# nuclia/nucliadb

Measured on AMD Instinct MI355X. Metric: queries/sec + recall@10 (768-dim cosine k-NN, HNSW M=30 ef=30 ef_upper=4 build_ef_upper=4, k=10), higher is better.
Workload: dtype f32

## Files before the change

### include/nidx_gpu.h

```cpp
#ifndef NIDX_GPU_H
#define NIDX_GPU_H

#include <stddef.h>
#include <stdint.h>

#ifdef __cplusplus
extern "C" {
#endif

#define NIDX_OK 0
#define NIDX_ERR_IO (-1)
#define NIDX_ERR_INCONSISTENT_DIMENSIONS (-2)
#define NIDX_ERR_INVALID_CONFIGURATION (-3)
#define NIDX_ERR_EMPTY_MERGE (-4)
#define NIDX_ERR_INVALID_ARGUMENT (-5)
#define NIDX_ERR_UNSUPPORTED (-6)
#define NIDX_ERR_DEVICE (-7)
#define NIDX_ERR_INVALID_GRAPH (-8)
#define NIDX_ERR_INEXACT (-9)
#define NIDX_ERR_OUT_OF_MEMORY (-10)
#define NIDX_ERR_INTERNAL (-11)
#define NIDX_ERR_BUSY (-12)

int32_t nidx_gpu_last_error(char *buf, size_t len);
// ... 168 lines not shown
int32_t nidx_gpu_vector_search_filtered_per_query(nidx_gpu_vector_index_t *index, const float *queries, uint32_t n_queries,
                                                  uint32_t query_dimension, const nidx_gpu_vector_search_params_t *params,
                                                  const nidx_gpu_filter_program_t *programs, uint32_t n_filters,
                                                  const uint32_t *filter_of_query, uint32_t *out_segment, uint32_t *out_paragraph,
                                                  uint32_t *out_vector, float *out_score, uint32_t *out_count, int32_t *out_method,
                                                  uint64_t *out_matching);

int32_t nidx_gpu_vector_segment_search_device(nidx_gpu_vector_index_t *index, uint32_t segment,
                                              const float *d_queries, uint32_t n_queries,
                                              const nidx_gpu_vector_search_params_t *params,
                                              const uint64_t *d_filter, uint32_t *d_out_vector,
                                              float *d_out_score, uint32_t *d_out_count, uint32_t *d_stats,
                                              void *stream);

int32_t nidx_gpu_vector_device_flags(nidx_gpu_vector_index_t *index, void *stream, uint32_t *flags_out);

int32_t nidx_gpu_vector_segment_search_device_exact(nidx_gpu_vector_index_t *index, uint32_t segment, const float *d_queries,
                                                    uint32_t n_queries, const nidx_gpu_vector_search_params_t *params,
                                                    const uint64_t *d_filter, uint32_t *d_out_block, uint32_t *host_out_block,
                                                    void *stream, uint32_t *n_retried_out);

int32_t nidx_gpu_diag_gather(const float *d_rows, uint32_t n_rows, uint32_t dimension, uint32_t waves, uint32_t gathers_per_wave,
                             int32_t rows_in_flight, uint32_t repeats, float *ms_out);

int32_t nidx_gpu_diag_single_query_latency(nidx_gpu_vector_index_t *index, const float *queries, uint32_t n_queries, uint32_t dimension,
                                           const nidx_gpu_vector_search_params_t *params, uint32_t threads, uint32_t calls,
                                           float *latencies_us_out, double *elapsed_s_out);

int32_t nidx_gpu_vector_search_submit(nidx_gpu_vector_index_t *index, const float *queries, uint32_t n_queries, uint32_t query_dimension,
                                      const nidx_gpu_vector_search_params_t *params, const uint64_t *const *segment_filters,
                                      uint64_t *ticket_out);
int32_t nidx_gpu_vector_search_wait(nidx_gpu_vector_index_t *index, uint64_t ticket, uint32_t *out_segment, uint32_t *out_paragraph,
                                    uint32_t *out_vector, float *out_score, uint32_t *out_count, uint32_t *n_retried_out);
int32_t nidx_gpu_vector_search_submit_filtered_per_query(nidx_gpu_vector_index_t *index, const float *queries, uint32_t n_queries,
                                                         uint32_t query_dimension, const nidx_gpu_vector_search_params_t *params,
                                                         const nidx_gpu_filter_program_t *programs, uint32_t n_filters,
                                                         const uint32_t *filter_of_query, uint64_t *ticket_out);

int32_t nidx_gpu_vector_search_submit_filtered_per_query_async(nidx_gpu_vector_index_t *index, const float *queries, uint32_t n_queries,
                                                               uint32_t query_dimension, const nidx_gpu_vector_search_params_t *params,
                                                               const nidx_gpu_filter_program_t *programs, uint32_t n_filters,
                                                               const uint32_t *filter_of_query, uint64_t *ticket_out);
int32_t nidx_gpu_vector_search_wait_routed(nidx_gpu_vector_index_t *index, uint64_t ticket, uint32_t *out_segment, uint32_t *out_paragraph,
                                           uint32_t *out_vector, float *out_score, uint32_t *out_count, int32_t *out_method,
                                           uint64_t *out_matching, uint32_t *n_retried_out);
int32_t nidx_gpu_use_hnsw_threshold(uint64_t total_nodes, uint64_t top_k, int32_t has_rabitq, uint64_t *threshold_out);
// ... 532 lines not shown
```

### nucliadb_amd/_lib.py

```python
from __future__ import annotations

import ctypes as C
import os

_HERE = os.path.dirname(os.path.abspath(__file__))
LIB_PATH = os.environ.get("NIDX_GPU_LIB") or os.path.join(_HERE, "libnidx_gpu.so")

NIDX_OK = 0
NIDX_ERR_IO = -1
NIDX_ERR_INCONSISTENT_DIMENSIONS = -2
NIDX_ERR_INVALID_CONFIGURATION = -3
NIDX_ERR_EMPTY_MERGE = -4
NIDX_ERR_INVALID_ARGUMENT = -5
NIDX_ERR_UNSUPPORTED = -6
NIDX_ERR_DEVICE = -7
NIDX_ERR_INVALID_GRAPH = -8
NIDX_ERR_INEXACT = -9
NIDX_ERR_OUT_OF_MEMORY = -10
NIDX_ERR_INTERNAL = -11
NIDX_ERR_BUSY = -12

SIMILARITY_DOT, SIMILARITY_COSINE = 0, 1
METHOD_AUTO, METHOD_HNSW, METHOD_BRUTE_FORCE, METHOD_BRUTE_FORCE_MFMA, METHOD_BRUTE_FORCE_BF16 = 0, 1, 2, 3, 4
METHOD_RABITQ_HNSW, METHOD_RABITQ_BRUTE_FORCE = 5, 6
# ... 306 lines not shown
    "nidx_gpu_vector_generation": (C.c_int32, [C.c_void_p, C.POINTER(C.c_uint64)]),
    "nidx_gpu_vector_set_tunable": (C.c_int32, [C.c_void_p, C.c_char_p, C.c_int32]),
    "nidx_gpu_vector_space_usage": (C.c_int32, [C.c_void_p, C.POINTER(C.c_uint64)]),
    "nidx_gpu_vector_num_segments": (C.c_int32, [C.c_void_p, C.POINTER(C.c_uint32)]),
    "nidx_gpu_vector_segment_records": (C.c_int32, [C.c_void_p, C.c_uint32, C.POINTER(C.c_uint32)]),
    "nidx_gpu_vector_search": (C.c_int32, [C.c_void_p, C.c_void_p, C.c_uint32, C.POINTER(VectorSearchParamsC), C.c_void_p,
                                           C.c_void_p, C.c_void_p, C.c_void_p, C.c_void_p, C.c_void_p, C.c_void_p]),
    "nidx_gpu_vector_search_dim": (C.c_int32, [C.c_void_p, C.c_void_p, C.c_uint32, C.c_uint32, C.POINTER(VectorSearchParamsC),
                                               C.c_void_p, C.c_void_p, C.c_void_p, C.c_void_p, C.c_void_p, C.c_void_p, C.c_void_p]),
    "nidx_gpu_vector_set_filter_index": (C.c_int32, [C.c_void_p, C.c_uint32, C.POINTER(FilterIndexC)]),
    "nidx_gpu_vector_search_filtered": (C.c_int32, [C.c_void_p, C.c_void_p, C.c_uint32, C.c_uint32, C.POINTER(VectorSearchParamsC),
                                                    C.c_void_p, C.c_void_p, C.c_void_p, C.c_void_p, C.c_void_p, C.c_void_p, C.c_void_p,
                                                    C.c_void_p]),
    "nidx_gpu_vector_segment_search_device": (C.c_int32, [C.c_void_p, C.c_uint32, C.c_void_p, C.c_uint32,
                                                          C.POINTER(VectorSearchParamsC), C.c_void_p, C.c_void_p, C.c_void_p,
                                                          C.c_void_p, C.c_void_p, C.c_void_p]),
    "nidx_gpu_bm25_apply_deletions": (C.c_int32, [C.c_void_p, C.c_uint32, C.c_void_p, C.c_uint32, C.POINTER(C.c_uint64)]),
    "nidx_gpu_vector_set_filter_keys": (C.c_int32, [C.c_void_p, C.c_uint32, C.c_void_p, C.c_void_p, C.c_uint32]),
    "nidx_gpu_vector_lookup_filter_keys": (C.c_int32, [C.c_void_p, C.c_uint32, C.c_void_p, C.c_void_p, C.c_void_p, C.c_uint32, C.c_void_p, C.c_void_p]),
    "nidx_gpu_diag_single_query_latency": (C.c_int32, [C.c_void_p, C.c_void_p, C.c_uint32, C.c_uint32, C.POINTER(VectorSearchParamsC), C.c_uint32,
                                                       C.c_uint32, C.c_void_p, C.POINTER(C.c_double)]),
    "nidx_gpu_diag_gather": (C.c_int32, [C.c_void_p, C.c_uint32, C.c_uint32, C.c_uint32, C.c_uint32, C.c_int32, C.c_uint32,
                                         C.POINTER(C.c_float)]),
    "nidx_gpu_vector_device_flags": (C.c_int32, [C.c_void_p, C.c_void_p, C.POINTER(C.c_uint32)]),
    "nidx_gpu_vector_segment_search_device_exact": (C.c_int32, [C.c_void_p, C.c_uint32, C.c_void_p, C.c_uint32,
                                                                C.POINTER(VectorSearchParamsC), C.c_void_p, C.c_void_p, C.c_void_p,
                                                                C.c_void_p, C.POINTER(C.c_uint32)]),
    "nidx_gpu_vector_search_one": (C.c_int32, [C.c_void_p, C.c_void_p, C.c_uint32, C.POINTER(VectorSearchParamsC), C.c_void_p,
                                               C.c_void_p, C.c_void_p, C.c_void_p, C.POINTER(C.c_uint32)]),
    "nidx_gpu_vector_search_submit": (C.c_int32, [C.c_void_p, C.c_void_p, C.c_uint32, C.c_uint32, C.POINTER(VectorSearchParamsC), C.c_void_p,
                                                  C.POINTER(C.c_uint64)]),
    "nidx_gpu_vector_search_wait": (C.c_int32, [C.c_void_p, C.c_uint64, C.c_void_p, C.c_void_p, C.c_void_p, C.c_void_p, C.c_void_p,
                                                C.POINTER(C.c_uint32)]),
    "nidx_gpu_vector_search_filtered_per_query": (C.c_int32, [C.c_void_p, C.c_void_p, C.c_uint32, C.c_uint32, C.POINTER(VectorSearchParamsC),
                                                              C.c_void_p, C.c_uint32, C.c_void_p, C.c_void_p, C.c_void_p, C.c_void_p,
                                                              C.c_void_p, C.c_void_p, C.c_void_p, C.c_void_p]),
    "nidx_gpu_vector_search_submit_filtered_per_query": (C.c_int32, [C.c_void_p, C.c_void_p, C.c_uint32, C.c_uint32,
                                                                     C.POINTER(VectorSearchParamsC), C.c_void_p, C.c_uint32, C.c_void_p,
                                                                     C.POINTER(C.c_uint64)]),
    "nidx_gpu_vector_search_submit_filtered_per_query_async": (C.c_int32, [C.c_void_p, C.c_void_p, C.c_uint32, C.c_uint32,
                                                                           C.POINTER(VectorSearchParamsC), C.c_void_p, C.c_uint32, C.c_void_p,
                                                                           C.POINTER(C.c_uint64)]),
    "nidx_gpu_vector_search_wait_routed": (C.c_int32, [C.c_void_p, C.c_uint64, C.c_void_p, C.c_void_p, C.c_void_p, C.c_void_p, C.c_void_p,
                                                       C.c_void_p, C.c_void_p, C.POINTER(C.c_uint32)]),
    "nidx_gpu_use_hnsw_threshold": (C.c_int32, [C.c_uint64, C.c_uint64, C.c_int32, C.POINTER(C.c_uint64)]),
    "nidx_gpu_vector_routed_stats": (C.c_int32, [C.c_void_p, C.POINTER(VectorRoutedStatsC)]),
# ... 195 lines not shown
```

### nucliadb_amd/csrc/hnsw_device.h

```cpp
#pragma once
#include "device_common.h"
#include "kernels.h"

namespace nidx {

#define NIDX_POOL_CAP 512
#define NIDX_VIS_EMPTY 0xffffffffu
#define NIDX_DEFER_CAP 256

struct NbBuf {
    uint32_t addr[64];
    float ab[64];
    float xx[64];
};
struct SearchShared {
    uint64_t pool[NIDX_POOL_CAP];
    NbBuf nb[2];
    uint32_t eps[256];
    int ctrl[12];
};

template <int NJ>
struct QueryRegs {
    float4 qv[NJ];
    float qq;
    double sqrt_qq;
};

template <int NJ>
__device__ inline void load_query(QueryRegs<NJ> &q, const float *qrow, uint32_t dp, int lane, bool cosine) {
    float acc = 0.f;
#pragma unroll
    for (int j = 0; j < NJ; j++) {
        q.qv[j] = load_row_chunk(qrow, dp, j, lane);
        acc = fma4(q.qv[j], q.qv[j], acc);
    }
    q.qq = wave_butterfly_sum(acc);
    q.sqrt_qq = cosine ? sqrt((double)q.qq) : 0.0;
}

__device__ inline float score_from_sums(float ab, float xx, float qq, double sqrt_qq, bool cosine) {
    if (!cosine) return ab;
    double dab = (double)ab, dxx = (double)xx;
// ... 224 lines not shown
template <int NJ, int EVR>
__device__ inline void eval_neighbours(const SegDev &seg, const QueryRegs<NJ> &q, NbBuf &nb, int n, bool cosine) {
    const int lane = threadIdx.x & 63;
    const int wave = nidx_tid() >> 6;
    const int nwaves = blockDim.x >> 6;
    for (int base = wave * EVR; base < n; base += nwaves * EVR) eval_row_group<NJ, EVR>(seg, q, nb, base, n, cosine, lane);
}

template <int NJ, int EVR>
__device__ inline void eval_neighbours_dynamic(const SegDev &seg, const QueryRegs<NJ> &q, NbBuf &nb, int n, bool cosine, int *next_row) {
    const int lane = threadIdx.x & 63;
    for (;;) {
        int base = 0;
        if (lane == 0) base = atomicAdd(next_row, EVR);
        base = __builtin_amdgcn_readfirstlane(base);
        if (base >= n) break;
        eval_row_group<NJ, EVR>(seg, q, nb, base, n, cosine, lane);
    }
}

#define NIDX_CMD_EVAL 0
#define NIDX_CMD_CLEAR 1
#define NIDX_CMD_EXIT 2
__device__ inline void split_post(SearchShared &sh, int op, int p, int n, int lane) {
    if (lane == 0) {
        sh.ctrl[0] = op | (p << 2) | (n << 3);
        sh.ctrl[3] = 0;
    }
    lds_barrier();
}
__device__ inline void split_close() { lds_barrier(); }
__device__ inline uint32_t load_edge_word(const GraphDev &g, uint32_t node, int layer, int lane, uint32_t &deg) {
    uint32_t w = 0;
    if (layer == 0) {
        w = g.l0[(size_t)node * NIDX_L0_STRIDE + lane];
    } else {
        uint32_t base = g.upper_base[node];
        if (base != 0xffffffffu && lane < NIDX_UP_STRIDE) w = g.upper[((size_t)base + (layer - 1)) * NIDX_UP_STRIDE + lane];
    }
    deg = lane_bcast_u32(w, 0);
    return w;
}

template <int NJ, int EVR>
__device__ inline void split_worker_loop(const SegDev &seg, const QueryRegs<NJ> &q, SearchShared &sh, uint32_t *vis, uint32_t vis_cap, bool cosine) {
    for (;;) {
        lds_barrier();
        const int cmd = __builtin_amdgcn_readfirstlane(sh.ctrl[0]);
        const int op = cmd & 3;
        if (op == NIDX_CMD_EVAL) eval_neighbours_dynamic<NJ, EVR>(seg, q, sh.nb[(cmd >> 2) & 1], cmd >> 3, cosine, &sh.ctrl[3]);
        else if (op == NIDX_CMD_CLEAR) vis_clear(vis, vis_cap);
        lds_barrier();
        if (op == NIDX_CMD_EXIT) return;
    }
}

#define NIDX_PARK_SLOTS 4
#define NIDX_EPS_BARE 0
#define NIDX_EPS_PARKED 1
#define NIDX_EPS_CARRIED 2
template <int NJ, int EFL, int EVR, bool SPLIT = false>
__device__ inline void layer_search_block(const SegDev &seg, const GraphDev &g, int layer, int k,
                                          const QueryRegs<NJ> &q, SearchShared &sh, uint32_t *vis, uint32_t vis_log2,
                                          WaveTopK<EFL> &res, SearchCounters &st, int ep_mode = NIDX_EPS_BARE) {
    const int lane = threadIdx.x & 63;
    const bool ctl = SPLIT ? true : (nidx_tid() >> 6) == 0;
    const bool cosine = seg.similarity == 1;
    const uint32_t vis_cap = 1u << vis_log2;
    const bool carried = ep_mode == NIDX_EPS_CARRIED;
    int pool_len = 0;
    uint32_t vis_count = 0;

    if constexpr (SPLIT) {
        split_post(sh, NIDX_CMD_CLEAR, 0, 0, lane);
        vis_clear(vis, vis_cap);
        split_close();
    } else {
        vis_clear(vis, vis_cap);
        __syncthreads();
    }
    int n_new = sh.ctrl[2];
    if (n_new > k) k = n_new < 64 * EFL ? n_new : 64 * EFL;
    CandSet<EFL> cand;
    cand.init();
    const int n_eps = carried ? 0 : n_new;
    uint32_t ptag = 0xffffffffu, pbase = 0xffffffffu;
// ... 196 lines not shown
            }
            if constexpr (SPLIT) split_post(sh, NIDX_CMD_EVAL, p ^ 1, n_next_reg, lane);
            else lds_barrier();
            const uint64_t t_b = clock64();
            st.cyc_ctl += t_b - t_a;
            const bool has_next = SPLIT ? false : sh.ctrl[5] != 0;
            const int n_next = SPLIT ? n_next_reg : sh.ctrl[6 + (p ^ 1)];
            if (!ctl && has_next) eval_neighbours_dynamic<NJ, EVR>(seg, q, nb_next, n_next, cosine, &sh.ctrl[3]);
            if (ctl) {
                while (todo) {
                    float ws = res.worst_score();
                    if (res.len >= k) {
                        todo &= __ballot(s > ws);
                        if (!todo) break;
                    }
                    int j = __ffsll((long long)todo) - 1;
                    todo &= ~(1ull << j);
                    float sj = lane_bcast_f32(s, j);
                    if (sj > ws || res.len < k) {
                        uint64_t ek;
                        bool eu;
                        cand.insert(res, rank_key(sj, lane_bcast_u32(addr, j)), k, lane, ek, eu);
                        if (eu && ek != NIDX_EMPTY_KEY && !(rank_key_score(ek) < res.worst_score())) {
                            if (pool_len == NIDX_POOL_CAP) {
                                pool_prune(sh.pool, pool_len, res.worst_score(), lane);
                                if (pool_len == NIDX_POOL_CAP) {
                                    st.flags |= NIDX_FLAG_POOL_INEXACT;
                                    pool_len--;
                                }
                            }
                            if (lane == 0) sh.pool[pool_len] = ek;
                            pool_len++;
                        }
                    }
                }
                int redo = 0;
                cont = 0;
                if (overflow) {
                    st.flags |= NIDX_FLAG_VISITED_OVERFLOW;
                } else {
                    cur = cand.pop(res);
                    if (cur == NIDX_EMPTY_KEY && pool_len > 0) cur = pool_pop(sh.pool, pool_len, lane);
                    cont = cur != NIDX_EMPTY_KEY && !(rank_key_score(cur) < res.worst_score());
                    redo = cont && cur != nxt;
                }
                redo_reg = redo;
                if (!SPLIT && lane == 0) {
                    sh.ctrl[0] = cont;
                    sh.ctrl[4] = redo;
// ... 42 lines not shown
```

### nucliadb_amd/csrc/hnsw_search.hip

```cpp
#include "hnsw_device.h"

namespace nidx {

template <int NJ>
__device__ inline bool rows_equal(const SegDev &seg, uint32_t a, uint32_t b, int lane) {
    const float *ra = seg.vectors + (size_t)a * seg.dp, *rb = seg.vectors + (size_t)b * seg.dp;
    bool eq = true;
#pragma unroll
    for (int j = 0; j < NJ; j++) {
        uint32_t e = (uint32_t)j * 256u + (uint32_t)lane * 4u;
        if (e < seg.dp) {
            uint4 x = *reinterpret_cast<const uint4 *>(ra + e);
            uint4 y = *reinterpret_cast<const uint4 *>(rb + e);
            eq = eq && x.x == y.x && x.y == y.y && x.z == y.z && x.w == y.w;
        }
    }
    return __all(eq);
}

template <int NJ, int EVR, int EFL, bool SPLIT>
__device__ __forceinline__ void hnsw_search_body(const HnswSearchArgs &a, const uint32_t qi, unsigned char *smem) {
    SearchShared &sh = *reinterpret_cast<SearchShared *>(smem);
    uint32_t *vis = reinterpret_cast<uint32_t *>(smem + sizeof(SearchShared));
    __shared__ uint32_t res_addr[64 * EFL];
    __shared__ float res_score[64 * EFL];
    __shared__ uint32_t res_para[64 * EFL];

    const int lane = threadIdx.x & 63;
    const bool cosine = a.seg.similarity == 1;
    const int k = (int)a.k;

    QueryRegs<NJ> q;
    load_query<NJ>(q, a.queries + (size_t)qi * a.seg.dp, a.seg.dp, lane, cosine);
    if constexpr (SPLIT) {
        if ((nidx_tid() >> 6) != 0) {
            split_worker_loop<NJ, EVR>(a.seg, q, sh, vis, 1u << a.vis_log2, cosine);
            return;
        }
    }
    const bool ctl = SPLIT ? true : (nidx_tid() >> 6) == 0;
    const uint64_t *filter = a.filter;
    if (a.filter_row) {
        const uint32_t row = a.filter_row[qi];
        filter = row == NIDX_FILTER_ROW_NONE ? nullptr : a.filter_table + (size_t)row * a.filter_words;
    }

    SearchCounters st = {0, 0, 0, 0, 0, 0, 0};
    const uint64_t t_start = clock64();
    WaveTopK<EFL> res;
// ... 25 lines not shown
                    a.dump_score[(size_t)qi * NIDX_DUMP_STRIDE + e] = rank_key_score(key);
                }
            }
            if (lane == 0) {
                a.dump_count[qi] = (uint32_t)res.len;
                if (a.stats) a.stats[(size_t)qi * NIDX_STAT_STRIDE + NIDX_STAT_FLAGS] = st.flags;
                if (st.flags && a.flag_word) atomicOr(a.flag_word, st.flags);
                if (a.flag_rows) a.flag_rows[qi] = st.flags;
            }
        }
        if constexpr (SPLIT) {
            split_post(sh, NIDX_CMD_EXIT, 0, 0, lane);
            split_close();
        }
        return;
    }

    const uint32_t vis_cap = 1u << a.vis_log2;
    int n_res = 0;
    bool scan_done = false;
    if (a.stats == nullptr && !entry_mode) {
        if (ctl) {
            bool done = false;
            if (res.len > 0 && st.flags == 0 && sh.ctrl[2] <= ef && ef + NIDX_DEFER_CAP <= NIDX_POOL_CAP) {
                const float s0 = rank_key_score(res.at(0)), ws = res.worst_score();
                if (s0 == s0 && ws == ws) {
                    uint32_t mp[EFL], mok[EFL];
#pragma unroll
                    for (int i = 0; i < EFL; i++) {
                        mp[i] = 0;
                        mok[i] = 0;
                        if (64 * i + lane < res.len) {
                            const uint32_t c = rank_key_addr(res.mine(i));
                            const uint32_t p = a.seg.para_of_vec ? a.seg.para_of_vec[c] : c;
                            mp[i] = p;
                            mok[i] = (!a.seg.alive || bit_test(a.seg.alive, p)) && (!filter || bit_test(filter, p));
                        }
                    }
                    int expansions = 0;
                    for (int r = 0; r < res.len; r++) {
                        const uint64_t ck = res.at(r);
                        const float cs = rank_key_score(ck);
                        const uint32_t c = rank_key_addr(ck);
                        if (!(cs > ws)) break;
                        if (cs < a.min_score) {
                            done = true;
                            break;
// ... 61 lines not shown
            const uint32_t addr = a.entry_vec[(size_t)qi * k + i];
            vis_insert(vis, a.vis_log2, addr);
            sh.pool[i] = rank_key(a.entry_score[(size_t)qi * k + i], addr);
        }
        pool_len = n_entry;
        vis_count = n_entry;
        if (lane == 0) {
            sh.ctrl[9] = -1;
            sh.ctrl[10] = 0;
        }
    } else if (ctl && !from_set) {
#pragma unroll
        for (int i = 0; i < EFL; i++) {
            uint64_t key = res.mine(i);
            if (64 * i + lane < res.len) {
                vis_insert(vis, a.vis_log2, rank_key_addr(key));
                sh.pool[64 * i + lane] = key;
            }
        }
        pool_len = res.len;
        vis_count = res.len;
        bool lazy = false;
        float ws = 0.f;
        if (res.len > 0 && st.flags == 0 && sh.ctrl[2] <= ef && ef + NIDX_DEFER_CAP <= NIDX_POOL_CAP) {
            const float s0 = rank_key_score(res.at(0));
            ws = res.worst_score();
            lazy = s0 == s0 && ws == ws;
        }
        if (lane == 0) {
            sh.ctrl[8] = __builtin_bit_cast(int, ws);
            sh.ctrl[9] = lazy ? 0 : -1;
            sh.ctrl[10] = 0;
        }
    }
    while (!from_set) {
        int cont = 1, n_new = 0;
        if (ctl) {
            int from = 0;
            const int waiting = sh.ctrl[10];
            if (waiting > 0) {
                n_new = waiting;
                from = sh.ctrl[11];
            } else for (;;) {
                cont = 0;
                n_new = 0;
                bool again = false;
                uint64_t ck = pool_pop(sh.pool, pool_len, lane);
// ... 91 lines not shown
            n_new = n_new > 64 ? 64 : n_new;
        }
        if constexpr (SPLIT) {
            if (!cont) break;
            if (n_new > 0) {
                split_post(sh, NIDX_CMD_EVAL, 0, n_new, lane);
                split_close();
            }
        } else {
            __syncthreads();
            if (!sh.ctrl[0]) break;
            n_new = sh.ctrl[1];
            eval_neighbours<NJ, EVR>(a.seg, q, sh.nb[0], n_new, cosine);
            __syncthreads();
        }
        if (ctl && n_new > 0) {
            float s = lane < n_new ? score_from_sums(sh.nb[0].ab[lane], sh.nb[0].xx[lane], q.qq, q.sqrt_qq, cosine) : 0.f;
            uint32_t addr = sh.nb[0].addr[lane];
            unsigned long long todo = __ballot(lane < n_new && s >= a.min_score);
            while (todo) {
                int j = __ffsll((long long)todo) - 1;
                todo &= todo - 1;
                uint64_t nk = rank_key(lane_bcast_f32(s, j), lane_bcast_u32(addr, j));
                if (pool_len == NIDX_POOL_CAP) {
                    uint64_t worst = ~0ull;
                    for (int i = lane; i < pool_len; i += 64) worst = sh.pool[i] < worst ? sh.pool[i] : worst;
                    worst = wave_min_u64(worst);
                    if (nk < worst) {
                        dropped_best = nk > dropped_best ? nk : dropped_best;
                        continue;
                    }
                    dropped_best = worst > dropped_best ? worst : dropped_best;
                    int idx = 0x7fffffff;
                    for (int i = lane; i < pool_len; i += 64)
                        if (sh.pool[i] == worst && i < idx) idx = i;
                    idx = wave_min_i32(idx);
                    if (lane == 0) sh.pool[idx] = nk;
                } else {
                    if (lane == 0) sh.pool[pool_len] = nk;
                    pool_len++;
                }
            }
        }
    }

    if constexpr (SPLIT) {
        split_post(sh, NIDX_CMD_EXIT, 0, 0, lane);
// ... 20 lines not shown
            }
        }
        if (lane == 0) {
            a.out_count[qi] = (uint32_t)n_res;
            if (st.flags && a.flag_word) atomicOr(a.flag_word, st.flags);
            if (a.flag_rows) a.flag_rows[qi] = st.flags;
            if (a.stats && entry_mode) {
                a.stats[(size_t)qi * NIDX_STAT_STRIDE + NIDX_STAT_FLAGS] |= st.flags;
            } else if (a.stats) {
                uint32_t *o = a.stats + (size_t)qi * NIDX_STAT_STRIDE;
                o[NIDX_STAT_EVALS] = st.evals;
                o[NIDX_STAT_EXPANSIONS] = st.expansions;
                o[NIDX_STAT_VISITED] = st.visited;
                o[NIDX_STAT_FLAGS] = st.flags;
                o[NIDX_STAT_CYC_CTL] = (uint32_t)st.cyc_ctl;
                o[NIDX_STAT_EDGE_HITS] = st.edge_hits;
                o[NIDX_STAT_CYC_INS] = (uint32_t)st.cyc_ins;
                o[NIDX_STAT_CYC_TOTAL] = (uint32_t)(clock64() - t_start);
            }
        }
    }
}

template <int NJ, int EVR, int MINW, int EFL, bool SPLIT>
__global__ __launch_bounds__(256, MINW) void hnsw_search_kernel(HnswSearchArgs a) {
    extern __shared__ __attribute__((aligned(16))) unsigned char smem[];
    hnsw_search_body<NJ, EVR, EFL, SPLIT>(a, blockIdx.x, smem);
}

template <int NJ, int EVR, int MINW, int EFL, bool SPLIT>
__global__ __launch_bounds__(256, MINW) void hnsw_search_segments_kernel(const HnswSearchArgs *__restrict__ table, uint32_t nq) {
    extern __shared__ __attribute__((aligned(16))) unsigned char smem[];
    const uint32_t s = blockIdx.x / nq;
    const HnswSearchArgs a = table[s];
    hnsw_search_body<NJ, EVR, EFL, SPLIT>(a, blockIdx.x - s * nq, smem);
}

template <int NJ, int EVR, int MINW, int EFL, bool SPLIT>
__global__ __launch_bounds__(256, MINW) void hnsw_search_routed_kernel(const HnswSearchArgs *__restrict__ table, const uint32_t *__restrict__ items,
                                                                       const uint32_t *__restrict__ n_items, uint32_t nq) {
    extern __shared__ __attribute__((aligned(16))) unsigned char smem[];
    const uint32_t s = blockIdx.x / nq, i = blockIdx.x - s * nq;
    if (i >= n_items[s]) return;
    const HnswSearchArgs a = table[s];
    hnsw_search_body<NJ, EVR, EFL, SPLIT>(a, items[(size_t)s * nq + i], smem);
}

template <int NJ, int EVR, int MINW, int EFL, bool SPLIT>
static hipError_t launch_form(const HnswSearchArgs &a, int waves, hipStream_t s) {
    if (a.seg_table && a.route_items) {
        size_t smem = sizeof(SearchShared) + ((size_t)4 << a.vis_log2);
        hipError_t e = hipFuncSetAttribute(reinterpret_cast<const void *>(&hnsw_search_routed_kernel<NJ, EVR, MINW, EFL, SPLIT>),
                                           hipFuncAttributeMaxDynamicSharedMemorySize, (int)smem);
        if (e != hipSuccess) return e;
        hipLaunchKernelGGL((hnsw_search_routed_kernel<NJ, EVR, MINW, EFL, SPLIT>), dim3(a.n_queries * a.n_table), dim3(64 * waves), smem, s,
                           a.seg_table, a.route_items, a.route_n_items, a.n_queries);
        return hipGetLastError();
    }
    if (a.seg_table) {
        size_t smem = sizeof(SearchShared) + ((size_t)4 << a.vis_log2);
        hipError_t e = hipFuncSetAttribute(reinterpret_cast<const void *>(&hnsw_search_segments_kernel<NJ, EVR, MINW, EFL, SPLIT>),
                                           hipFuncAttributeMaxDynamicSharedMemorySize, (int)smem);
        if (e != hipSuccess) return e;
        hipLaunchKernelGGL((hnsw_search_segments_kernel<NJ, EVR, MINW, EFL, SPLIT>), dim3(a.n_queries * a.n_table), dim3(64 * waves), smem, s,
                           a.seg_table, a.n_queries);
        return hipGetLastError();
    }
    size_t smem = sizeof(SearchShared) + ((size_t)4 << a.vis_log2);
    hipError_t e = hipFuncSetAttribute(reinterpret_cast<const void *>(&hnsw_search_kernel<NJ, EVR, MINW, EFL, SPLIT>),
                                       hipFuncAttributeMaxDynamicSharedMemorySize, (int)smem);
    if (e != hipSuccess) return e;
    hipLaunchKernelGGL((hnsw_search_kernel<NJ, EVR, MINW, EFL, SPLIT>), dim3(a.n_queries), dim3(64 * waves), smem, s, a);
    return hipGetLastError();
}

template <int NJ, int EVR, int MINW, int EFL>
static hipError_t launch_v(const HnswSearchArgs &a, int waves, hipStream_t s) {
    return waves >= 2 ? launch_form<NJ, EVR, MINW, EFL, true>(a, waves, s) : launch_form<NJ, EVR, MINW, EFL, false>(a, waves, s);
}

static uint32_t layer0_ef(const HnswSearchArgs &a) {
    const uint32_t efs = a.ef_search ? a.ef_search : NIDX_EF_SEARCH;
    return a.k > efs ? a.k : efs;
}

template <int NJ>
hipError_t launch_nj(const HnswSearchArgs &a, int waves, hipStream_t s) {
    const uint32_t ef = layer0_ef(a);
    if (ef > 256) return launch_v<NJ, 2, 2, 8>(a, waves, s);
    if (ef > 128) return launch_v<NJ, 2, 2, 4>(a, waves, s);
    if (ef > 64) return launch_v<NJ, 2, 2, 2>(a, waves, s);
    if (a.min_waves >= 6) return launch_v<NJ, 2, 6, 1>(a, waves, s);
    if (a.min_waves == 5) return a.eval_rows == 4 ? launch_v<NJ, 4, 5, 1>(a, waves, s) : launch_v<NJ, 2, 5, 1>(a, waves, s);
    if (a.eval_rows == 3) return a.min_waves >= 4 ? launch_v<NJ, 3, 4, 1>(a, waves, s) : launch_v<NJ, 3, 2, 1>(a, waves, s);
    if (a.eval_rows == 2) return a.min_waves >= 4 ? launch_v<NJ, 2, 4, 1>(a, waves, s) : launch_v<NJ, 2, 2, 1>(a, waves, s);
    return a.min_waves >= 4 ? launch_v<NJ, 4, 4, 1>(a, waves, s) : launch_v<NJ, 4, 2, 1>(a, waves, s);
}

#if NIDX_HNSW_PART != 0
template hipError_t launch_nj<NIDX_HNSW_PART>(const HnswSearchArgs &, int, hipStream_t);
#else
extern template hipError_t launch_nj<1>(const HnswSearchArgs &, int, hipStream_t);
extern template hipError_t launch_nj<2>(const HnswSearchArgs &, int, hipStream_t);
extern template hipError_t launch_nj<3>(const HnswSearchArgs &, int, hipStream_t);
extern template hipError_t launch_nj<4>(const HnswSearchArgs &, int, hipStream_t);

template <int NJ>
static hipError_t launch_wide(const HnswSearchArgs &a, int waves, hipStream_t s) {
    const uint32_t ef = layer0_ef(a);
    if (ef > 256) return launch_v<NJ, 2, 1, 8>(a, waves, s);
    if (ef > 128) return launch_v<NJ, 2, 1, 4>(a, waves, s);
    if (ef > 64) return launch_v<NJ, 2, 1, 2>(a, waves, s);
    return launch_v<NJ, 2, 1, 1>(a, waves, s);
}
// ... 21 lines not shown
```

### nucliadb_amd/csrc/json_index.cpp

```cpp
#include <string.h>

#include <atomic>
#include <memory>
#include <mutex>

#include "json_plan.h"
#include "kernels.h"
#include "prefilter_handover.h"

using namespace nidx;

namespace {
struct JsonColumn {
    uint64_t n_values = 0;
    DevBuf docs, values;
};
struct JsonSegment {
    uint32_t n_docs = 0;
    std::vector<JsonColumn> columns;
};
std::atomic<uint64_t> g_json_index_uid{1};

struct JsonIndex {
    int device = 0;
// ... 26 lines not shown
struct JsonResourceLink {
    int device = 0;
    uint64_t index_uid = 0, text_generation = 0, n_resources = 0, linked_documents = 0;
    PrefilterRowLayout layout;
    DevBuf doc_resource;
};

uint64_t list_bits(const std::vector<uint64_t> &host, uint32_t *out, uint64_t capacity) {
    uint64_t n = 0;
    for (size_t w = 0; w < host.size(); w++)
        for (uint64_t v = host[w]; v; v &= v - 1) {
            if (n < capacity) out[n] = (uint32_t)(w * 64 + (size_t)__builtin_ctzll(v));
            n++;
        }
    return n;
}
}

extern "C" {

int32_t nidx_gpu_json_open(const nidx_gpu_json_segment_t *segments, uint32_t n_segments, nidx_gpu_json_index_t **index_out,
                           nidx_gpu_json_open_stats_t *stats_out) try {
    if (!index_out || (n_segments && !segments)) return fail(NIDX_ERR_INVALID_ARGUMENT, "NULL argument");
    uint64_t total_docs = 0;
    for (uint32_t s = 0; s < n_segments; s++) {
        const nidx_gpu_json_segment_t &sg = segments[s];
        if (sg.n_docs && !sg.resource_ids) return fail(NIDX_ERR_INVALID_ARGUMENT, "segment %u: NULL resource ids", s);
        if (sg.n_columns && !sg.columns) return fail(NIDX_ERR_INVALID_ARGUMENT, "segment %u: NULL columns", s);
        total_docs += sg.n_docs;
        for (uint32_t c = 0; c < sg.n_columns; c++) {
            const nidx_gpu_json_column_t &col = sg.columns[c];
            if (col.type < NIDX_JSON_STR || col.type > NIDX_JSON_DATE) return fail(NIDX_ERR_INVALID_ARGUMENT, "segment %u column %u: unknown type %d", s, c, col.type);
            if ((col.path_len && !col.path) || (col.n_values && (!col.docs || !col.values)))
                return fail(NIDX_ERR_INVALID_ARGUMENT, "segment %u column %u: NULL path, docs or values", s, c);
            if (col.type == NIDX_JSON_STR && (!col.dict_offsets || (col.n_dict && col.dict_offsets[col.n_dict] && !col.dict_bytes)))
                return fail(NIDX_ERR_INVALID_ARGUMENT, "segment %u column %u: a STR column without its dictionary", s, c);
            for (uint64_t i = 0; i < col.n_values; i++) {
                if (col.docs[i] >= sg.n_docs) return fail(NIDX_ERR_INVALID_ARGUMENT, "segment %u column %u: document %u of %u", s, c, col.docs[i], sg.n_docs);
                if (i && col.docs[i] < col.docs[i - 1]) return fail(NIDX_ERR_INVALID_ARGUMENT, "segment %u column %u: docs descend at value %llu", s, c, (unsigned long long)i);
                if (col.type == NIDX_JSON_STR && col.values[i] >= col.n_dict)
                    return fail(NIDX_ERR_INVALID_ARGUMENT, "segment %u column %u: ordinal %llu of %u", s, c, (unsigned long long)col.values[i], col.n_dict);
            }
        }
    }
    if (total_docs + 64ull * n_segments >= (1ull << 31)) return fail(NIDX_ERR_UNSUPPORTED, "a JSON index of 2^31 documents or more");
    std::unique_ptr<JsonIndex> idx(new JsonIndex());
// ... 478 lines not shown
```

### nucliadb_amd/csrc/vector_index.cpp

```cpp
#include <math.h>
#include <stdio.h>
#include <stdlib.h>
#include <string.h>

#include <algorithm>
#include <unordered_map>
#include <chrono>
#include <memory>
#include <mutex>

#include "device_common.h"
#include "hnsw_graph.h"
#include "host_common.h"
#include "kernels.h"
#include "vector_index.h"
#include "prefilter_handover.h"

namespace nidx {

static thread_local char g_last_error[512];

static void record_error(const char *fmt, va_list ap) { vsnprintf(g_last_error, sizeof(g_last_error), fmt, ap); }

void set_error(const char *fmt, ...) {
// ... 2133 lines not shown
    *count_out = n;
    return NIDX_OK;
} NIDX_ABI_CATCH

int32_t nidx_gpu_set_device(int32_t device) try {
    NIDX_HIP(hipSetDevice(device));
    return NIDX_OK;
} NIDX_ABI_CATCH

int32_t nidx_gpu_vector_open(const nidx_gpu_vector_config_t *config, const nidx_gpu_vector_segment_t *segments,
                             uint32_t n_segments, nidx_gpu_vector_index_t **index_out) try {
    if (!config || !index_out || (n_segments && !segments)) return fail(NIDX_ERR_INVALID_ARGUMENT, "NULL argument");
    *index_out = nullptr;
    if (config->dimension == 0) return fail(NIDX_ERR_INVALID_CONFIGURATION, "Invalid configuration: Vector dimension cannot be 0");
    if (config->similarity != NIDX_SIMILARITY_DOT && config->similarity != NIDX_SIMILARITY_COSINE)
        return fail(NIDX_ERR_INVALID_CONFIGURATION, "Invalid configuration: unknown similarity %d", config->similarity);
    if (config->vector_cardinality != NIDX_CARDINALITY_SINGLE && config->vector_cardinality != NIDX_CARDINALITY_MULTI)
        return fail(NIDX_ERR_INVALID_CONFIGURATION, "unknown vector cardinality %d", config->vector_cardinality);
    if (config->dimension > 4096) return fail(NIDX_ERR_UNSUPPORTED, "dimension > 4096 is not supported (got %u)", config->dimension);
    std::unique_ptr<VectorIndex> idx(new VectorIndex());
    idx->cfg = *config;
    if (const char *e = getenv("NIDX_GPU_WAVES_PER_QUERY")) idx->waves_per_query = std::max(1, std::min(4, atoi(e)));
    if (const char *e = getenv("NIDX_GPU_EVAL_ROWS")) { idx->eval_rows = std::max(2, std::min(4, atoi(e))); idx->shape_pinned = true; }
    if (const char *e = getenv("NIDX_GPU_MIN_WAVES")) { idx->min_waves = atoi(e) >= 4 ? std::min(6, atoi(e)) : 2; idx->shape_pinned = true; }
    if (const char *e = getenv("NIDX_GPU_VIS_LOG2")) { idx->default_vis_log2 = (uint32_t)std::max(10, std::min(15, atoi(e))); idx->vis_pinned = true; }
    if (const char *e = getenv("NIDX_GPU_BUILD_VIS_LOG2")) {
        idx->build_vis_log2 = (uint32_t)std::max(10, std::min(15, atoi(e)));
        idx->build_vis_pinned = true;
    }
    NIDX_HIP(hipGetDevice(&idx->device));
    NIDX_HIP(hipStreamCreateWithFlags(&idx->stream, hipStreamNonBlocking));
    NIDX_HIP(idx->flag_word.alloc(64));
    NIDX_HIP(hipMemset(idx->flag_word.p, 0, 64));
    NIDX_HIP(idx->pin_flag.reserve(64));
    idx->segs.resize(n_segments);
    for (uint32_t s = 0; s < n_segments; s++) {
        int32_t rc = open_segment(*config, segments[s], idx->segs[s], idx->stream);
        if (rc != NIDX_OK) return rc;
    }
    *index_out = reinterpret_cast<nidx_gpu_vector_index_t *>(idx.release());
    return NIDX_OK;
} NIDX_ABI_CATCH

void nidx_gpu_vector_close(nidx_gpu_vector_index_t *index) {
    VectorIndex *idx = reinterpret_cast<VectorIndex *>(index);
    if (!idx) return;
    (void)hipSetDevice(idx->device);
    delete idx;
}

int32_t nidx_gpu_vector_sync(nidx_gpu_vector_index_t *index, const nidx_gpu_vector_sync_entry_t *entries, uint32_t n_entries,
                             const uint8_t *deletion_prefix_bytes, const uint64_t *deletion_prefix_offsets,
                             const int64_t *deletion_seqs, uint32_t n_deletions, uint32_t timeout_ms,
                             nidx_gpu_vector_sync_stats_t *stats_out) try {
    VectorIndex *idx = reinterpret_cast<VectorIndex *>(index);
    if (!idx || (n_entries && !entries) || (n_deletions && (!deletion_prefix_offsets || !deletion_seqs)))
        return fail(NIDX_ERR_INVALID_ARGUMENT, "NULL argument");
    return idx->sync(entries, n_entries, deletion_prefix_bytes, deletion_prefix_offsets, deletion_seqs, n_deletions, timeout_ms, stats_out);
} NIDX_ABI_CATCH

int32_t nidx_gpu_vector_generation(const nidx_gpu_vector_index_t *index, uint64_t *generation_out) try {
    const VectorIndex *idx = reinterpret_cast<const VectorIndex *>(index);
    if (!idx || !generation_out) return fail(NIDX_ERR_INVALID_ARGUMENT, "NULL argument");
    *generation_out = idx->gate.generation.load(std::memory_order_seq_cst);
    return NIDX_OK;
} NIDX_ABI_CATCH

int32_t nidx_gpu_vector_set_tunable(nidx_gpu_vector_index_t *index, const char *name, int32_t value) try {
    VectorIndex *idx = reinterpret_cast<VectorIndex *>(index);
    if (!idx || !name) return fail(NIDX_ERR_INVALID_ARGUMENT, "NULL argument");
    std::lock_guard<std::mutex> lock(idx->mu);
    std::string n(name);
    if (n == "waves_per_query") idx->waves_per_query = std::max(1, std::min(4, (int)value));
    else if (n == "eval_rows") { idx->eval_rows = std::max(2, std::min(4, (int)value)); idx->shape_pinned = true; }
    else if (n == "min_waves") { idx->min_waves = value >= 4 ? std::min(6, (int)value) : 2; idx->shape_pinned = true; }
    else if (n == "launch_shape") idx->launch_shape = (int)std::max<int64_t>(0, std::min<int64_t>(2, (int64_t)value));
    else if (n == "vis_log2") { idx->default_vis_log2 = (uint32_t)std::max(10, std::min(15, (int)value)); idx->vis_pinned = true; }
    else if (n == "coalesce_window_us") idx->coalescer_config(value, -1, -1);
    else if (n == "coalesce_max_batch") idx->coalescer_config(-1, value, -1);
    else if (n == "coalesce_in_flight") idx->coalescer_config(-1, -1, value);
    else if (n == "coalesce_max_callers") idx->coalescer_admission(std::max(0, (int)value), -1);
    else if (n == "coalesce_reject_when_full") idx->coalescer_admission(-1, value != 0);
    else if (n == "pipeline_depth") idx->pipeline_config(value);
    else if (n == "pipeline_walks") idx->pipeline_config(-1, value);
    else if (n == "stage_threads") set_stage_threads(value);
    else if (n == "closest_prefetch") idx->closest_prefetch = value != 0;
    else if (n == "per_query_filter_scratch_kib") idx->pq_scratch_cap = value > 0 ? (uint64_t)value << 10 : 1ull << 30;
    else if (n == "serial_segments") idx->serial_segments = value != 0;
    else if (n == "build_vis_log2") { idx->build_vis_log2 = (uint32_t)std::max(10, std::min(15, (int)value)); idx->build_vis_pinned = true; }
    else if (n == "ef_search") {
        if (value < 0 || value > NIDX_K_MAX) return fail(NIDX_ERR_INVALID_ARGUMENT, "ef_search must be in 0..%d", NIDX_K_MAX);
        idx->ef_search = (uint32_t)value;
    }
    else if (n == "build_ef_upper") {
        if (value < 0 || value > 64) return fail(NIDX_ERR_INVALID_ARGUMENT, "build_ef_upper must be in 0..64");
        idx->build_ef_upper = (uint32_t)value;
    }
    else if (n == "ef_upper") {
// ... 401 lines not shown
```

### nucliadb_amd/csrc/vector_index.h

```cpp
#pragma once
#include <atomic>
#include <condition_variable>
#include <memory>
#include <mutex>
#include <vector>

#include "hnsw_graph.h"
#include "host_common.h"
#include "kernels.h"

namespace nidx {

bool use_hnsw(uint64_t total_nodes, uint64_t matching_nodes, uint64_t top_k, bool has_rabitq);
void normalize_row(const float *in, float *out, uint32_t d);
void stage_query_rows(const float *src, float *dst, uint32_t nq, uint32_t d, uint32_t dp, bool normalize);
void set_stage_threads(int32_t n);

struct VectorSegment {
    uint32_t n = 0, dim = 0, dp = 0, n_paragraphs = 0;
    DevBuf vectors;
    DevBuf norm2;
    DevBuf norm2_serial;
    DevBuf vectors16;
    uint32_t dp16 = 0;
// ... 100 lines not shown
            (void)hipStreamDestroy(stream);
        }
        if (sync_stream) {
            (void)hipStreamSynchronize(sync_stream);
            (void)hipStreamDestroy(sync_stream);
        }
        if (scratch_event) (void)hipEventDestroy(scratch_event);
        pipe.reset();
    }
    std::mutex mu;
    std::vector<VectorSegment> segs;
    mutable GenGate gate;
    std::mutex sync_mu;
    hipStream_t sync_stream = nullptr;
    DevBuf sync_dev;
    PinBuf sync_pin;
    int32_t sync(const nidx_gpu_vector_sync_entry_t *entries, uint32_t n_entries, const uint8_t *del_bytes, const uint64_t *del_offsets,
                 const int64_t *del_seqs, uint32_t n_deletions, uint32_t timeout_ms, nidx_gpu_vector_sync_stats_t *stats_out);
    int waves_per_query = 4;
    int eval_rows = 4;
    int min_waves = 4;
    bool shape_pinned = false;
    int rows_for(uint32_t nq) const { return (!shape_pinned && nq <= 256) ? 4 : (shape_pinned && min_waves >= 5) ? 2 : eval_rows; }
    int waves_for(uint32_t nq) const { return (!shape_pinned && nq <= 256) ? 2 : (!shape_pinned && crowded_now()) ? 5 : min_waves; }
    static bool crowded_launch();
    static void set_crowded_launch(bool on);
    int launch_shape = 0;
    bool crowded_now() const { return launch_shape == 1 || (launch_shape == 0 && crowded_launch()); }
    bool vis_pinned = false;
    uint32_t vis_for(uint32_t nq) const { return (!vis_pinned && !shape_pinned && nq > 256 && crowded_now()) ? std::min<uint32_t>(default_vis_log2, 12u) : default_vis_log2; }
    uint32_t ef_search = 0;
    uint32_t ef_upper = 0;
    bool closest_prefetch = true;
    bool serial_segments = false;
    uint32_t default_vis_log2 = 13;
    uint32_t build_vis_log2 = 14;
    bool build_vis_pinned = false;
    uint32_t build_ef_upper = 0;
    uint32_t last_build_flags = 0;
    uint32_t last_build_escalated_at = 0;
    uint64_t last_build_stats[8] = {0, 0, 0, 0, 0, 0, 0, 0};
    DevBuf scratch_fstack, scratch_flists, scratch_fcount, scratch_q16, scratch_cand_vec, scratch_cand_score, scratch_cand_count, scratch_multi_vec, scratch_multi_score, scratch_multi_count, scratch_qnorm, scratch_partial, scratch_queries, scratch_filter, scratch_out_vec, scratch_out_score, scratch_out_count,
        scratch_stats, scratch_rq, scratch_planes, scratch_vis, scratch_ties, scratch_entry_vec, scratch_entry_score, scratch_entry_count,
        scratch_dump_vec, scratch_dump_score, scratch_dump_count, scratch_spill_pool, scratch_spill_cmax, scratch_spill_vis, scratch_spill_ids, scratch_rowmask, scratch_floor, scratch_floor2, scratch_bf16_flags, scratch_bf16_counts;
    uint64_t scan_matching_hint = ~0ull;
    const uint32_t *pq_filter_row = nullptr;
    const uint64_t *pq_filter_table = nullptr;
// ... 109 lines not shown
```

Measured before the change: 4.542 million.

## Add compact LDS layout for seven-walk occupancy in crowded HNSW launches

Result: faster. 4.651 million (median of 6 runs) (+2.4%).

```diff
diff --git a/include/nidx_gpu.h b/include/nidx_gpu.h
--- a/include/nidx_gpu.h
+++ b/include/nidx_gpu.h
@@ -214,6 +214,9 @@
 
 int32_t nidx_gpu_diag_gather(const float *d_rows, uint32_t n_rows, uint32_t dimension, uint32_t waves, uint32_t gathers_per_wave,
                              int32_t rows_in_flight, uint32_t repeats, float *ms_out);
+
+int32_t nidx_gpu_diag_hnsw_launch_shape(int32_t min_waves_tunable, int32_t launch_shape, uint32_t n_queries, int32_t *eval_rows_out,
+                                        int32_t *min_waves_out, uint32_t *vis_log2_out);
 
 int32_t nidx_gpu_diag_single_query_latency(nidx_gpu_vector_index_t *index, const float *queries, uint32_t n_queries, uint32_t dimension,
                                            const nidx_gpu_vector_search_params_t *params, uint32_t threads, uint32_t calls,
diff --git a/nucliadb_amd/_lib.py b/nucliadb_amd/_lib.py
--- a/nucliadb_amd/_lib.py
+++ b/nucliadb_amd/_lib.py
@@ -352,6 +352,8 @@
                                                        C.c_uint32, C.c_void_p, C.POINTER(C.c_double)]),
     "nidx_gpu_diag_gather": (C.c_int32, [C.c_void_p, C.c_uint32, C.c_uint32, C.c_uint32, C.c_uint32, C.c_int32, C.c_uint32,
                                          C.POINTER(C.c_float)]),
+    "nidx_gpu_diag_hnsw_launch_shape": (C.c_int32, [C.c_int32, C.c_int32, C.c_uint32, C.POINTER(C.c_int32), C.POINTER(C.c_int32),
+                                                    C.POINTER(C.c_uint32)]),
     "nidx_gpu_vector_device_flags": (C.c_int32, [C.c_void_p, C.c_void_p, C.POINTER(C.c_uint32)]),
     "nidx_gpu_vector_segment_search_device_exact": (C.c_int32, [C.c_void_p, C.c_uint32, C.c_void_p, C.c_uint32,
                                                                 C.POINTER(VectorSearchParamsC), C.c_void_p, C.c_void_p, C.c_void_p,
diff --git a/nucliadb_amd/csrc/hnsw_device.h b/nucliadb_amd/csrc/hnsw_device.h
--- a/nucliadb_amd/csrc/hnsw_device.h
+++ b/nucliadb_amd/csrc/hnsw_device.h
@@ -18,7 +18,21 @@
     NbBuf nb[2];
     uint32_t eps[256];
     int ctrl[12];
+    static constexpr int POOL_CAP = NIDX_POOL_CAP;
+    static constexpr bool RES_ON_NB1 = false;
 };
+#define NIDX_POOL_CAP_COMPACT 432
+struct SearchSharedCompact {
+    NbBuf nb[2];
+    uint32_t eps[256];
+    int ctrl[12];
+    uint64_t pool[NIDX_POOL_CAP_COMPACT];
+    static constexpr int POOL_CAP = NIDX_POOL_CAP_COMPACT;
+    static constexpr bool RES_ON_NB1 = true;
+};
+static_assert(sizeof(SearchSharedCompact) + (4u << 12) <= 22528, "the compact walk must leave room for seven walks per CU");
+static_assert(64 + NIDX_DEFER_CAP <= NIDX_POOL_CAP_COMPACT, "closest_up_nodes' deferral must fit the compact pool (ef <= 64)");
+static_assert(sizeof(SearchSharedCompact) % 16 == 0 && sizeof(SearchShared) % 16 == 0, "the visited table follows the block");
 
 template <int NJ>
 struct QueryRegs {
@@ -289,7 +303,8 @@
 #define NIDX_CMD_EVAL 0
 #define NIDX_CMD_CLEAR 1
 #define NIDX_CMD_EXIT 2
-__device__ inline void split_post(SearchShared &sh, int op, int p, int n, int lane) {
+template <class SH>
+__device__ inline void split_post(SH &sh, int op, int p, int n, int lane) {
     if (lane == 0) {
         sh.ctrl[0] = op | (p << 2) | (n << 3);
         sh.ctrl[3] = 0;
@@ -309,8 +324,8 @@
     return w;
 }
 
-template <int NJ, int EVR>
-__device__ inline void split_worker_loop(const SegDev &seg, const QueryRegs<NJ> &q, SearchShared &sh, uint32_t *vis, uint32_t vis_cap, bool cosine) {
+template <int NJ, int EVR, class SH>
+__device__ inline void split_worker_loop(const SegDev &seg, const QueryRegs<NJ> &q, SH &sh, uint32_t *vis, uint32_t vis_cap, bool cosine) {
     for (;;) {
         lds_barrier();
         const int cmd = __builtin_amdgcn_readfirstlane(sh.ctrl[0]);
@@ -326,9 +341,9 @@
 #define NIDX_EPS_BARE 0
 #define NIDX_EPS_PARKED 1
 #define NIDX_EPS_CARRIED 2
-template <int NJ, int EFL, int EVR, bool SPLIT = false>
+template <int NJ, int EFL, int EVR, bool SPLIT = false, class SH = SearchShared>
 __device__ inline void layer_search_block(const SegDev &seg, const GraphDev &g, int layer, int k,
-                                          const QueryRegs<NJ> &q, SearchShared &sh, uint32_t *vis, uint32_t vis_log2,
+                                          const QueryRegs<NJ> &q, SH &sh, uint32_t *vis, uint32_t vis_log2,
                                           WaveTopK<EFL> &res, SearchCounters &st, int ep_mode = NIDX_EPS_BARE) {
     const int lane = threadIdx.x & 63;
     const bool ctl = SPLIT ? true : (nidx_tid() >> 6) == 0;
@@ -571,9 +586,9 @@
                         bool eu;
                         cand.insert(res, rank_key(sj, lane_bcast_u32(addr, j)), k, lane, ek, eu);
                         if (eu && ek != NIDX_EMPTY_KEY && !(rank_key_score(ek) < res.worst_score())) {
-                            if (pool_len == NIDX_POOL_CAP) {
+                            if (pool_len == SH::POOL_CAP) {
                                 pool_prune(sh.pool, pool_len, res.worst_score(), lane);
-                                if (pool_len == NIDX_POOL_CAP) {
+                                if (pool_len == SH::POOL_CAP) {
                                     st.flags |= NIDX_FLAG_POOL_INEXACT;
                                     pool_len--;
                                 }
diff --git a/nucliadb_amd/csrc/hnsw_search.hip b/nucliadb_amd/csrc/hnsw_search.hip
--- a/nucliadb_amd/csrc/hnsw_search.hip
+++ b/nucliadb_amd/csrc/hnsw_search.hip
@@ -1,3 +1,7 @@
+#include <atomic>
+#include <mutex>
+#include <type_traits>
+
 #include "hnsw_device.h"
 
 namespace nidx {
@@ -18,13 +22,36 @@
     return __all(eq);
 }
 
-template <int NJ, int EVR, int EFL, bool SPLIT>
+template <int EFL, bool ON_NB1>
+struct HitArrays {
+    uint32_t *addr;
+    float *score;
+    uint32_t *para;
+    __device__ __forceinline__ explicit HitArrays(NbBuf &nb) {
+        if constexpr (ON_NB1) {
+            addr = nb.addr;
+            score = nb.ab;
+            para = reinterpret_cast<uint32_t *>(nb.xx);
+        } else {
+            __shared__ uint32_t s_addr[64 * EFL];
+            __shared__ float s_score[64 * EFL];
+            __shared__ uint32_t s_para[64 * EFL];
+            addr = s_addr;
+            score = s_score;
+            para = s_para;
+        }
+    }
+};
+
+template <int NJ, int EVR, int EFL, bool SPLIT, class SH>
 __device__ __forceinline__ void hnsw_search_body(const HnswSearchArgs &a, const uint32_t qi, unsigned char *smem) {
-    SearchShared &sh = *reinterpret_cast<SearchShared *>(smem);
-    uint32_t *vis = reinterpret_cast<uint32_t *>(smem + sizeof(SearchShared));
-    __shared__ uint32_t res_addr[64 * EFL];
-    __shared__ float res_score[64 * EFL];
-    __shared__ uint32_t res_para[64 * EFL];
+    SH &sh = *reinterpret_cast<SH *>(smem);
+    uint32_t *vis = reinterpret_cast<uint32_t *>(smem + sizeof(SH));
+    static_assert(!SH::RES_ON_NB1 || EFL == 1, "nb[1] holds the hits of one 64-entry list");
+    const HitArrays<EFL, SH::RES_ON_NB1> hits(sh.nb[1]);
+    uint32_t *const res_addr = hits.addr;
+    float *const res_score = hits.score;
+    uint32_t *const res_para = hits.para;
 
     const int lane = threadIdx.x & 63;
     const bool cosine = a.seg.similarity == 1;
@@ -96,7 +123,7 @@
     if (a.stats == nullptr && !entry_mode) {
         if (ctl) {
             bool done = false;
-            if (res.len > 0 && st.flags == 0 && sh.ctrl[2] <= ef && ef + NIDX_DEFER_CAP <= NIDX_POOL_CAP) {
+            if (res.len > 0 && st.flags == 0 && sh.ctrl[2] <= ef && ef + NIDX_DEFER_CAP <= SH::POOL_CAP) {
                 const float s0 = rank_key_score(res.at(0)), ws = res.worst_score();
                 if (s0 == s0 && ws == ws) {
                     uint32_t mp[EFL], mok[EFL];
@@ -204,7 +231,7 @@
         vis_count = res.len;
         bool lazy = false;
         float ws = 0.f;
-        if (res.len > 0 && st.flags == 0 && sh.ctrl[2] <= ef && ef + NIDX_DEFER_CAP <= NIDX_POOL_CAP) {
+        if (res.len > 0 && st.flags == 0 && sh.ctrl[2] <= ef && ef + NIDX_DEFER_CAP <= SH::POOL_CAP) {
             const float s0 = rank_key_score(res.at(0));
             ws = res.worst_score();
             lazy = s0 == s0 && ws == ws;
@@ -342,7 +369,7 @@
                 int j = __ffsll((long long)todo) - 1;
                 todo &= todo - 1;
                 uint64_t nk = rank_key(lane_bcast_f32(s, j), lane_bcast_u32(addr, j));
-                if (pool_len == NIDX_POOL_CAP) {
+                if (pool_len == SH::POOL_CAP) {
                     uint64_t worst = ~0ull;
                     for (int i = lane; i < pool_len; i += 64) worst = sh.pool[i] < worst ? sh.pool[i] : worst;
                     worst = wave_min_u64(worst);
@@ -409,10 +436,13 @@
     }
 }
 
+template <int MINW>
+using SharedOf = std::conditional_t<MINW >= 7, SearchSharedCompact, SearchShared>;
+
 template <int NJ, int EVR, int MINW, int EFL, bool SPLIT>
 __global__ __launch_bounds__(256, MINW) void hnsw_search_kernel(HnswSearchArgs a) {
     extern __shared__ __attribute__((aligned(16))) unsigned char smem[];
-    hnsw_search_body<NJ, EVR, EFL, SPLIT>(a, blockIdx.x, smem);
+    hnsw_search_body<NJ, EVR, EFL, SPLIT, SharedOf<MINW>>(a, blockIdx.x, smem);
 }
 
 template <int NJ, int EVR, int MINW, int EFL, bool SPLIT>
@@ -420,7 +450,7 @@
     extern __shared__ __attribute__((aligned(16))) unsigned char smem[];
     const uint32_t s = blockIdx.x / nq;
     const HnswSearchArgs a = table[s];
-    hnsw_search_body<NJ, EVR, EFL, SPLIT>(a, blockIdx.x - s * nq, smem);
+    hnsw_search_body<NJ, EVR, EFL, SPLIT, SharedOf<MINW>>(a, blockIdx.x - s * nq, smem);
 }
 
 template <int NJ, int EVR, int MINW, int EFL, bool SPLIT>
@@ -430,32 +460,51 @@
     const uint32_t s = blockIdx.x / nq, i = blockIdx.x - s * nq;
     if (i >= n_items[s]) return;
     const HnswSearchArgs a = table[s];
-    hnsw_search_body<NJ, EVR, EFL, SPLIT>(a, items[(size_t)s * nq + i], smem);
-}
+    hnsw_search_body<NJ, EVR, EFL, SPLIT, SharedOf<MINW>>(a, items[(size_t)s * nq + i], smem);
+}
+
+struct DynLdsLimit {
+    static constexpr int MAX_DEVICES = 64;
+    std::atomic<int> set_to[MAX_DEVICES];
+    std::mutex mu;
+    DynLdsLimit() {
+        for (auto &v : set_to) v.store(0, std::memory_order_relaxed);
+    }
+    hipError_t ensure(const void *kernel, size_t bytes) {
+        int dev = 0;
+        hipError_t e = hipGetDevice(&dev);
+        if (e != hipSuccess) return e;
+        if (dev < 0 || dev >= MAX_DEVICES) return hipFuncSetAttribute(kernel, hipFuncAttributeMaxDynamicSharedMemorySize, (int)bytes);
+        if ((size_t)set_to[dev].load(std::memory_order_acquire) >= bytes) return hipSuccess;
+        std::lock_guard<std::mutex> lock(mu);
+        if ((size_t)set_to[dev].load(std::memory_order_relaxed) >= bytes) return hipSuccess;
+        e = hipFuncSetAttribute(kernel, hipFuncAttributeMaxDynamicSharedMemorySize, (int)bytes);
+        if (e == hipSuccess) set_to[dev].store((int)bytes, std::memory_order_release);
+        return e;
+    }
+};
 
 template <int NJ, int EVR, int MINW, int EFL, bool SPLIT>
 static hipError_t launch_form(const HnswSearchArgs &a, int waves, hipStream_t s) {
+    const size_t smem = sizeof(SharedOf<MINW>) + ((size_t)4 << a.vis_log2);
     if (a.seg_table && a.route_items) {
-        size_t smem = sizeof(SearchShared) + ((size_t)4 << a.vis_log2);
-        hipError_t e = hipFuncSetAttribute(reinterpret_cast<const void *>(&hnsw_search_routed_kernel<NJ, EVR, MINW, EFL, SPLIT>),
-                                           hipFuncAttributeMaxDynamicSharedMemorySize, (int)smem);
+        static DynLdsLimit limit;
+        hipError_t e = limit.ensure(reinterpret_cast<const void *>(&hnsw_search_routed_kernel<NJ, EVR, MINW, EFL, SPLIT>), smem);
         if (e != hipSuccess) return e;
         hipLaunchKernelGGL((hnsw_search_routed_kernel<NJ, EVR, MINW, EFL, SPLIT>), dim3(a.n_queries * a.n_table), dim3(64 * waves), smem, s,
                            a.seg_table, a.route_items, a.route_n_items, a.n_queries);
         return hipGetLastError();
     }
     if (a.seg_table) {
-        size_t smem = sizeof(SearchShared) + ((size_t)4 << a.vis_log2);
-        hipError_t e = hipFuncSetAttribute(reinterpret_cast<const void *>(&hnsw_search_segments_kernel<NJ, EVR, MINW, EFL, SPLIT>),
-                                           hipFuncAttributeMaxDynamicSharedMemorySize, (int)smem);
+        static DynLdsLimit limit;
+        hipError_t e = limit.ensure(reinterpret_cast<const void *>(&hnsw_search_segments_kernel<NJ, EVR, MINW, EFL, SPLIT>), smem);
         if (e != hipSuccess) return e;
         hipLaunchKernelGGL((hnsw_search_segments_kernel<NJ, EVR, MINW, EFL, SPLIT>), dim3(a.n_queries * a.n_table), dim3(64 * waves), smem, s,
                            a.seg_table, a.n_queries);
         return hipGetLastError();
     }
-    size_t smem = sizeof(SearchShared) + ((size_t)4 << a.vis_log2);
-    hipError_t e = hipFuncSetAttribute(reinterpret_cast<const void *>(&hnsw_search_kernel<NJ, EVR, MINW, EFL, SPLIT>),
-                                       hipFuncAttributeMaxDynamicSharedMemorySize, (int)smem);
+    static DynLdsLimit limit;
+    hipError_t e = limit.ensure(reinterpret_cast<const void *>(&hnsw_search_kernel<NJ, EVR, MINW, EFL, SPLIT>), smem);
     if (e != hipSuccess) return e;
     hipLaunchKernelGGL((hnsw_search_kernel<NJ, EVR, MINW, EFL, SPLIT>), dim3(a.n_queries), dim3(64 * waves), smem, s, a);
     return hipGetLastError();
@@ -477,6 +526,12 @@
     if (ef > 256) return launch_v<NJ, 2, 2, 8>(a, waves, s);
     if (ef > 128) return launch_v<NJ, 2, 2, 4>(a, waves, s);
     if (ef > 64) return launch_v<NJ, 2, 2, 2>(a, waves, s);
+    if (a.min_waves >= 7) {
+        if constexpr (NJ <= 3) {
+            if (waves >= 2) return launch_form<NJ, 4, 7, 1, true>(a, waves, s);
+        }
+        return launch_v<NJ, 4, 5, 1>(a, waves, s);
+    }
     if (a.min_waves >= 6) return launch_v<NJ, 2, 6, 1>(a, waves, s);
     if (a.min_waves == 5) return a.eval_rows == 4 ? launch_v<NJ, 4, 5, 1>(a, waves, s) : launch_v<NJ, 2, 5, 1>(a, waves, s);
     if (a.eval_rows == 3) return a.min_waves >= 4 ? launch_v<NJ, 3, 4, 1>(a, waves, s) : launch_v<NJ, 3, 2, 1>(a, waves, s);
diff --git a/nucliadb_amd/csrc/json_index.cpp b/nucliadb_amd/csrc/json_index.cpp
--- a/nucliadb_amd/csrc/json_index.cpp
+++ b/nucliadb_amd/csrc/json_index.cpp
@@ -72,6 +72,7 @@
 int32_t nidx_gpu_json_open(const nidx_gpu_json_segment_t *segments, uint32_t n_segments, nidx_gpu_json_index_t **index_out,
                            nidx_gpu_json_open_stats_t *stats_out) try {
     if (!index_out || (n_segments && !segments)) return fail(NIDX_ERR_INVALID_ARGUMENT, "NULL argument");
+    *index_out = nullptr;
     uint64_t total_docs = 0;
     for (uint32_t s = 0; s < n_segments; s++) {
         const nidx_gpu_json_segment_t &sg = segments[s];
diff --git a/nucliadb_amd/csrc/vector_index.cpp b/nucliadb_amd/csrc/vector_index.cpp
--- a/nucliadb_amd/csrc/vector_index.cpp
+++ b/nucliadb_amd/csrc/vector_index.cpp
@@ -2179,7 +2179,7 @@
     idx->cfg = *config;
     if (const char *e = getenv("NIDX_GPU_WAVES_PER_QUERY")) idx->waves_per_query = std::max(1, std::min(4, atoi(e)));
     if (const char *e = getenv("NIDX_GPU_EVAL_ROWS")) { idx->eval_rows = std::max(2, std::min(4, atoi(e))); idx->shape_pinned = true; }
-    if (const char *e = getenv("NIDX_GPU_MIN_WAVES")) { idx->min_waves = atoi(e) >= 4 ? std::min(6, atoi(e)) : 2; idx->shape_pinned = true; }
+    if (const char *e = getenv("NIDX_GPU_MIN_WAVES")) { idx->min_waves = VectorIndex::clamp_min_waves(atoi(e)); idx->shape_pinned = true; }
     if (const char *e = getenv("NIDX_GPU_VIS_LOG2")) { idx->default_vis_log2 = (uint32_t)std::max(10, std::min(15, atoi(e))); idx->vis_pinned = true; }
     if (const char *e = getenv("NIDX_GPU_BUILD_VIS_LOG2")) {
         idx->build_vis_log2 = (uint32_t)std::max(10, std::min(15, atoi(e)));
@@ -2223,6 +2223,21 @@
     return NIDX_OK;
 } NIDX_ABI_CATCH
 
+int32_t nidx_gpu_diag_hnsw_launch_shape(int32_t min_waves_tunable, int32_t launch_shape, uint32_t n_queries, int32_t *eval_rows_out,
+                                        int32_t *min_waves_out, uint32_t *vis_log2_out) try {
+    if (!eval_rows_out || !min_waves_out || !vis_log2_out) return fail(NIDX_ERR_INVALID_ARGUMENT, "NULL argument");
+    VectorIndex idx;
+    if (min_waves_tunable >= 0) {
+        idx.min_waves = VectorIndex::clamp_min_waves(min_waves_tunable);
+        idx.shape_pinned = true;
+    }
+    idx.launch_shape = std::max(0, std::min(2, (int)launch_shape));
+    *eval_rows_out = idx.rows_for(n_queries);
+    *min_waves_out = idx.waves_for(n_queries);
+    *vis_log2_out = idx.vis_for(n_queries);
+    return NIDX_OK;
+} NIDX_ABI_CATCH
+
 int32_t nidx_gpu_vector_set_tunable(nidx_gpu_vector_index_t *index, const char *name, int32_t value) try {
     VectorIndex *idx = reinterpret_cast<VectorIndex *>(index);
     if (!idx || !name) return fail(NIDX_ERR_INVALID_ARGUMENT, "NULL argument");
@@ -2230,7 +2245,7 @@
     std::string n(name);
     if (n == "waves_per_query") idx->waves_per_query = std::max(1, std::min(4, (int)value));
     else if (n == "eval_rows") { idx->eval_rows = std::max(2, std::min(4, (int)value)); idx->shape_pinned = true; }
-    else if (n == "min_waves") { idx->min_waves = value >= 4 ? std::min(6, (int)value) : 2; idx->shape_pinned = true; }
+    else if (n == "min_waves") { idx->min_waves = VectorIndex::clamp_min_waves((int)value); idx->shape_pinned = true; }
     else if (n == "launch_shape") idx->launch_shape = (int)std::max<int64_t>(0, std::min<int64_t>(2, (int64_t)value));
     else if (n == "vis_log2") { idx->default_vis_log2 = (uint32_t)std::max(10, std::min(15, (int)value)); idx->vis_pinned = true; }
     else if (n == "coalesce_window_us") idx->coalescer_config(value, -1, -1);
diff --git a/nucliadb_amd/csrc/vector_index.h b/nucliadb_amd/csrc/vector_index.h
--- a/nucliadb_amd/csrc/vector_index.h
+++ b/nucliadb_amd/csrc/vector_index.h
@@ -146,7 +146,8 @@
     int min_waves = 4;
     bool shape_pinned = false;
     int rows_for(uint32_t nq) const { return (!shape_pinned && nq <= 256) ? 4 : (shape_pinned && min_waves >= 5) ? 2 : eval_rows; }
-    int waves_for(uint32_t nq) const { return (!shape_pinned && nq <= 256) ? 2 : (!shape_pinned && crowded_now()) ? 5 : min_waves; }
+    int waves_for(uint32_t nq) const { return (!shape_pinned && nq <= 256) ? 2 : (!shape_pinned && crowded_now()) ? 7 : min_waves; }
+    static int clamp_min_waves(int v) { return v >= 4 ? std::min(7, v) : 2; }
     static bool crowded_launch();
     static void set_crowded_launch(bool on);
     int launch_shape = 0;
```
